# jinhan/tacotron2-vae

Hardware: AMD Instinct MI355X
Metric: mel-frames/s (train step, batch=6, 80-mel) (higher is better)
Workload: dtype f32; 1 GPU; configs[1]: Tacotron2-VAE fp32 train step (fwd+loss+bwd+clip+Adam), B=6/GPU fixed shape T_in=84 T_out=400, dropout on, random-init seed 1234; step_mode=hip-graph replay, decoder_forward=persistent, decoder_backward=persistent, startup_steps=43, global_batch=6, parallelism=dp1

## Files before the change

### tacotron2-vae_amd/csrc/conv_gemm.hip

```cpp
#include <stdlib.h>
#include <type_traits>
#include "t2v_common.h"
#include "t2v_kernels.h"
#include "t2v_ring.h"
#include "t2v_coop.h"
#include "t2v_x3.h"


#define CG_BM 64
#define CG_BN 64
#define CG_BK 32

struct ConvGemmArgs {
    const float* W;
    const float* X;
    const float* dY;
    const float* bias;
    float* Y;
    float* stat_part;
    int B, Cin, T, M, KS;
};

template <int MODE, int KS>
__global__ __launch_bounds__(256) void k_conv_gemm(ConvGemmArgs a) {
// ... 158 lines not shown
        if (second_ == 0u) return;
        if (tid == 0) __hip_atomic_store(a.ks_ctr + tile, 0u, __ATOMIC_RELAXED, __HIP_MEMORY_SCOPE_AGENT);
        const float* other = a.ks_part + (((1 - blockIdx.z) * ntile + tile) * 256 + tid) * (4 * NTW);
        float o[NTW][4];
#pragma unroll
        for (int n = 0; n < NTW; ++n)
#pragma unroll
            for (int r = 0; r < 4; ++r) o[n][r] = ld_sc1(other + 4 * n + r);
#pragma unroll
        for (int n = 0; n < NTW; ++n)
#pragma unroll
            for (int r = 0; r < 4; ++r) acc[n][r] += o[n][r];
    }
    float psum[4] = {0.f, 0.f, 0.f, 0.f}, psq[4] = {0.f, 0.f, 0.f, 0.f};
#pragma unroll
    for (int r = 0; r < 4; ++r) {
        const int m = m0 + 16 * wave + 4 * kq + r;
        if (m < a.M) {
            const float bv = a.bias ? a.bias[m] : 0.f;
            float* yrow = a.Y + ((size_t)bb * a.M + m) * a.T;
#pragma unroll
            for (int n = 0; n < NTW; ++n) {
                const int t = t0 + 16 * n + j;
                if (t < a.T) {
                    const float v = acc[n][r] + bv;
                    yrow[t] = v;
                    psum[r] += v;
                    psq[r] = fmaf(v, v, psq[r]);
                }
            }
        }
    }
    if (a.stat_part) {
#pragma unroll
        for (int r = 0; r < 4; ++r) {
            const float s1 = row16_sum(psum[r]), s2 = row16_sum(psq[r]);
            const int m = m0 + 16 * wave + 4 * kq + r;
            if (j == 0 && m < a.M) {
                float* dst = a.stat_part + ((size_t)blockIdx.x * a.M + m) * 2;
                dst[0] = s1;
                dst[1] = s2;
            }
        }
    }
}

template <int NTW>
__global__ __launch_bounds__(256) void k_conv5_fwd(ConvTiledArgs a) {
    constexpr int BN = 16 * NTW;
    constexpr int XW = BN + 4;
    constexpr int XS = BN == 32 ? 48 : BN <= 64 ? 80 : 112;
    constexpr int NX = (16 * XW + 255) / 256;
    __shared__ float As[2][CT_KT][CT_AS];
    __shared__ float Xs[2][16][XS];
    const int tid = threadIdx.x, wave = tid >> 6, lane = tid & 63;
    const int kq = lane >> 4, j = lane & 15;
    const int bb = blockIdx.x / a.tiles_per_item, t0 = (blockIdx.x % a.tiles_per_item) * BN;
    const int m0 = blockIdx.y * CT_BM;
    const int CK = a.Cin * 5;
    const int nkt_all = a.Cin / 16;
    const int kt0 = gridDim.z > 1 ? (int)blockIdx.z * (nkt_all / 2) : 0;
    const int nkt = gridDim.z > 1 ? (blockIdx.z == 0 ? nkt_all / 2 : nkt_all - nkt_all / 2) : nkt_all;

    const bool stamp = a.prof && tid == 0 && blockIdx.x == 0 && blockIdx.y == 0 && blockIdx.z == 0;
    if (stamp) { a.prof[0] = __builtin_readcyclecounter(); a.prof[2] = wall_clock64(); }
    float4 ra[5];
    float rx[NX];
    const int a_m = tid & 63, w4 = tid >> 6;
    const float* a_row = a.W + (size_t)min(m0 + a_m, a.M - 1) * CK + 4 * w4;
    int a_lds[20];
#pragma unroll
    for (int q = 0; q < 20; ++q) {
        const int k = 4 * w4 + 16 * (q >> 2) + (q & 3);
        const int c = k / 5, kx = k - 5 * c;
        a_lds[q] = (16 * kx + c) * CT_AS + a_m;
    }
    const float* x_item = a.X + (size_t)bb * a.Cin * a.T;
    int x_goff[NX], x_lds[NX];
    bool x_ok[NX];
#pragma unroll
    for (int i = 0; i < NX; ++i) {
        const int e = tid + 256 * i;
        const int c = min(e / XW, 15), jj = e - (e / XW) * XW;
        const int t = t0 - 2 + jj;
        x_ok[i] = e < 16 * XW && t >= 0 && t < a.T;
        x_goff[i] = c * a.T + min(max(t, 0), a.T - 1);
        x_lds[i] = e < 16 * XW ? c * XS + jj : -1;
    }
    auto load_one = [&](int kt, int q) {
        if (q < 5) {
            ra[q] = *(const float4*)(a_row + 80 * (kt0 + kt) + 16 * q);
        } else {
            const float v = x_item[(size_t)16 * (kt0 + kt) * a.T + x_goff[q - 5]];
            rx[q - 5] = x_ok[q - 5] ? v : 0.f;
        }
    };
    auto store_one = [&](int buf, int q) {
        if (q < 20) {
            const float4 v4 = ra[q >> 2];
            const float v = (q & 3) == 0 ? v4.x : (q & 3) == 1 ? v4.y : (q & 3) == 2 ? v4.z : v4.w;
            (&As[buf][0][0])[a_lds[q]] = v;
        } else if (q < 20 + NX) {
            if (x_lds[q - 20] >= 0) (&Xs[buf][0][0])[x_lds[q - 20]] = rx[q - 20];
        }
    };
    constexpr int NLOAD = 5 + NX, NSTORE = 20 + NX;
    constexpr int S_ST0 = 11;
    static_assert(NLOAD <= S_ST0 + 1 && NSTORE <= 3 * (20 - S_ST0), "side work must fit the k-steps");

    f32x4 acc[NTW];
#pragma unroll
    for (int n = 0; n < NTW; ++n) acc[n] = f32x4{0.f, 0.f, 0.f, 0.f};
#pragma unroll
    for (int q = 0; q < NLOAD; ++q) load_one(0, q);
#pragma unroll
    for (int q = 0; q < NSTORE; ++q) store_one(0, q);
    __syncthreads();
    for (int kt = 0; kt < nkt; ++kt) {
        const int buf = kt & 1;
        const int kn = min(kt + 1, nkt - 1);
        const float* ap = &As[buf][kq][16 * wave + j];
        const float* xp = &Xs[buf][kq][j];
        float av[2], bv[2][NTW];
        av[0] = ap[0];
#pragma unroll
        for (int n = 0; n < NTW; ++n) bv[0][n] = xp[16 * n];
#pragma unroll
        for (int s = 0; s < 20; ++s) {
            if (s < NLOAD) load_one(kn, s);
            if (s + 1 < 20) {
                av[(s + 1) & 1] = ap[4 * (s + 1) * CT_AS];
#pragma unroll
                for (int n = 0; n < NTW; ++n)
                    bv[(s + 1) & 1][n] = xp[4 * ((s + 1) & 3) * XS + 16 * n + ((s + 1) >> 2)];
            }
            __builtin_amdgcn_sched_barrier(0);
#pragma unroll
            for (int n = 0; n < NTW; ++n) acc[n] = mfma16x4(av[s & 1], bv[s & 1][n], acc[n]);
            __builtin_amdgcn_sched_barrier(0);
            if (s >= S_ST0) {
#pragma unroll
                for (int q = 3 * (s - S_ST0); q < 3 * (s - S_ST0) + 3; ++q) store_one(buf ^ 1, q);
                __builtin_amdgcn_sched_barrier(0);
            }
        }
        __syncthreads();
    }
    if (stamp) { a.prof[1] = __builtin_readcyclecounter(); a.prof[3] = wall_clock64(); }
    conv5_fwd_finish<NTW>(a, acc, bb, t0, m0);
}

#define CD_RING 3
#define CD_AS 84
__device__ float g_conv5_zero[4];

template <int NTW>
__global__ __launch_bounds__(256) void k_conv5_fwd_dma(ConvTiledArgs a) {
    constexpr int BN = 16 * NTW;
    constexpr int XW = BN + 4;
    constexpr int XS = BN == 32 ? 48 : BN <= 64 ? 80 : 112;
    constexpr int NXD = 16 * XS / 256;
    constexpr int G = 6 + NXD;
    constexpr int AST = CT_BM * CD_AS, STG = AST + 16 * XS;
    static_assert(16 * XS % 256 == 0 && AST % 256 == 0, "whole 64-lane requests");
    __shared__ __attribute__((aligned(16))) float lds_[CD_RING * STG];
    const unsigned lds0 = (unsigned)(unsigned long)(__attribute__((address_space(3))) void*)&lds_[0];
    const int tid = threadIdx.x, wave = __builtin_amdgcn_readfirstlane(tid >> 6), lane = tid & 63;
    const int kq = lane >> 4, j = lane & 15;
    const int bb = blockIdx.x / a.tiles_per_item, t0 = (blockIdx.x % a.tiles_per_item) * BN;
    const int m0 = blockIdx.y * CT_BM;
    const int CK = a.Cin * 5;
    const int nkt_all = a.Cin / 16;
    const int kt0 = gridDim.z > 1 ? (int)blockIdx.z * (nkt_all / 2) : 0;
    const int nkt = gridDim.z > 1 ? (blockIdx.z == 0 ? nkt_all / 2 : nkt_all - nkt_all / 2) : nkt_all;

    const bool stamp = a.prof && tid == 0 && blockIdx.x == 0 && blockIdx.y == 0 && blockIdx.z == 0;
    if (stamp) { a.prof[0] = __builtin_readcyclecounter(); a.prof[2] = wall_clock64(); }
    const float* a_ptr[6];
#pragma unroll
    for (int i = 0; i < 6; ++i) {
        const int u = 64 * min(wave + 4 * i, 20) + lane;
        const int row = u / 21, pc = u - 21 * row;
        a_ptr[i] = a.W + (size_t)min(m0 + row, a.M - 1) * CK + 80 * kt0 + 4 * min(pc, 19);
    }
    const float* x_ptr[NXD];
    size_t x_step[NXD];
#pragma unroll
    for (int i = 0; i < NXD; ++i) {
        const int e = 64 * (wave + 4 * i) + lane;
        const int c = e / XS, jj = e - c * XS;
        const int t = t0 - 2 + jj;
        const bool ok = jj < XW && t >= 0 && t < a.T;
        x_ptr[i] = ok ? a.X + ((size_t)bb * a.Cin + 16 * kt0 + c) * a.T + t : g_conv5_zero;
        x_step[i] = ok ? (size_t)16 * a.T : 0;
    }
    auto request = [&](unsigned dst, int q) {
        if (q < 5) {
            t2v_dma16(a_ptr[q], dst + 1024u * (unsigned)wave + 4096u * q);
            a_ptr[q] += 80;
        } else if (q == 5) {
            t2v_dma16(a_ptr[5], dst + 20480u);
            a_ptr[5] += 80;
        } else if (q < G) {
            t2v_dma4(x_ptr[q - 6], dst + 4u * AST + 256u * (unsigned)wave + 1024u * (q - 6));
            x_ptr[q - 6] += x_step[q - 6];
        }
    };

    f32x4 acc[NTW];
#pragma unroll
    for (int n = 0; n < NTW; ++n) acc[n] = f32x4{0.f, 0.f, 0.f, 0.f};
#pragma unroll
    for (int q = 0; q < G; ++q) request(lds0, q);
    if (nkt > 1) {
#pragma unroll
        for (int q = 0; q < G; ++q) request(lds0 + 4u * STG, q);
    }
    if (nkt > 1) t2v_wait_vmcnt<G>(); else t2v_wait_vmcnt<0>();
    __syncthreads();
    constexpr int CD_SYNC = 10;
    constexpr int TWO = G > 20 - CD_SYNC ? G - (20 - CD_SYNC) : 0;
    static_assert(G <= 2 * (20 - CD_SYNC) && (TWO == 0 || NTW >= 3), "a tile's requests fit the steps behind the barrier");
    const int lane_a = CD_AS * (16 * wave + j) + 5 * kq, lane_x = AST + kq * XS + j;
    float av[2], bv[2][NTW];
    auto fetch = [&](const float* ap, const float* xp, int s) {
        av[s & 1] = ap[20 * (s & 3) + (s >> 2)];
#pragma unroll
        for (int n = 0; n < NTW; ++n) bv[s & 1][n] = xp[4 * (s & 3) * XS + 16 * n + (s >> 2)];
    };
    auto tile = [&](auto more_c, const float* ap, const float* xp, const float* ap1, const float* xp1, unsigned dst2) {
        constexpr bool MORE = decltype(more_c)::value;
#pragma unroll
        for (int s = 0; s < 20; ++s) {
            if (s == CD_SYNC) {
                t2v_wait_vmcnt<0>();
                __syncthreads();
                __builtin_amdgcn_sched_barrier(0);
            }
            const int sr = s - CD_SYNC;
            const int q0 = !MORE || sr < 0 ? -1 : sr < TWO ? 2 * sr : sr + TWO;
            const int q1 = MORE && sr >= 0 && sr < TWO ? 2 * sr + 1 : -1;
#pragma unroll
            for (int n = 0; n < NTW; ++n) {
                acc[n] = mfma16x4(av[s & 1], bv[s & 1][n], acc[n]);
                __builtin_amdgcn_sched_barrier(0);
                if (n == 0) { if (s + 1 < 20) fetch(ap, xp, s + 1); else fetch(ap1, xp1, 0); }
                if (n == 1 && q0 >= 0 && q0 < G) request(dst2, q0);
                if (n == 2 && q1 >= 0) request(dst2, q1);
                __builtin_amdgcn_sched_barrier(0);
            }
        }
    };
    fetch(&lds_[lane_a], &lds_[lane_x], 0);
    int stg = 0;
    for (int kt = 0; kt < nkt; ++kt) {
        const int stg1 = stg == CD_RING - 1 ? 0 : stg + 1, stg2 = stg == 0 ? CD_RING - 1 : stg - 1;
        const float* ap = &lds_[stg * STG + lane_a];
        const float* xp = &lds_[stg * STG + lane_x];
        const float* ap1 = &lds_[stg1 * STG + lane_a];
        const float* xp1 = &lds_[stg1 * STG + lane_x];
        if (kt + 2 < nkt) tile(std::true_type{}, ap, xp, ap1, xp1, lds0 + 4u * (unsigned)(stg2 * STG));
        else tile(std::false_type{}, ap, xp, ap1, xp1, 0u);
        stg = stg1;
    }
    if (stamp) { a.prof[1] = __builtin_readcyclecounter(); a.prof[3] = wall_clock64(); }
    conv5_fwd_finish<NTW>(a, acc, bb, t0, m0);
}

template <int BT>
__global__ __launch_bounds__(256) void k_conv5_dw(ConvTiledArgs a) {
    constexpr int XW = BT + 4;
    constexpr int XS = (BT == 80) ? 100 : 116;
    constexpr int NA = BT / 16;
    constexpr int NX = (16 * XW + 255) / 256;
    __shared__ float As[2][BT][CT_AS];
    __shared__ float Xs[2][16][XS];
    const int tid = threadIdx.x, wave = tid >> 6, lane = tid & 63;
    const int kq = lane >> 4, j = lane & 15;
    const int c0 = blockIdx.x * 16, m0 = blockIdx.y * CT_BM;
    const int CK = a.Cin * 5;
    const int tiles = (a.T + BT - 1) / BT, nkt_all = a.B * tiles;
    const int per = (nkt_all + gridDim.z - 1) / gridDim.z;
    const int kt_lo = blockIdx.z * per, kt_hi = min(nkt_all, kt_lo + per);
    const bool vec = (a.T & 3) == 0;

    float4 ra[NA];
    float rx[NX];
    const int a_m = tid & 63;
    const bool a_ok = m0 + a_m < a.M;
    auto load_tiles = [&](int kt) {
        const int bb = kt / tiles, t0 = (kt - bb * tiles) * BT;
        const float* arow = a.dY + ((size_t)bb * a.M + (a_ok ? m0 + a_m : 0)) * a.T;
#pragma unroll
        for (int i = 0; i < NA; ++i) {
            const int t = t0 + 4 * ((tid >> 6) + 4 * i);
            float4 v = make_float4(0.f, 0.f, 0.f, 0.f);
            if (a_ok) {
                if (vec) {
                    if (t < a.T) v = *(const float4*)(arow + t);
                } else {
                    if (t < a.T) v.x = arow[t];
                    if (t + 1 < a.T) v.y = arow[t + 1];
                    if (t + 2 < a.T) v.z = arow[t + 2];
                    if (t + 3 < a.T) v.w = arow[t + 3];
                }
            }
            ra[i] = v;
        }
        const float* x_item = a.X + ((size_t)bb * a.Cin + c0) * a.T;
#pragma unroll
        for (int i = 0; i < NX; ++i) {
            const int e = tid + 256 * i;
            const int c = e / XW, jj = e - c * XW;
            const int t = t0 - 2 + jj;
            rx[i] = (c < 16 && t >= 0 && t < a.T) ? x_item[(size_t)c * a.T + t] : 0.f;
        }
    };
    auto store_tiles = [&](int buf) {
#pragma unroll
        for (int i = 0; i < NA; ++i) {
            const int k = 4 * ((tid >> 6) + 4 * i);
            As[buf][k][a_m] = ra[i].x;
            As[buf][k + 1][a_m] = ra[i].y;
            As[buf][k + 2][a_m] = ra[i].z;
            As[buf][k + 3][a_m] = ra[i].w;
        }
#pragma unroll
        for (int i = 0; i < NX; ++i) {
            const int e = tid + 256 * i;
            const int c = e / XW, jj = e - c * XW;
            if (c < 16) Xs[buf][c][jj] = rx[i];
        }
    };

    int boff[5];
#pragma unroll
    for (int n = 0; n < 5; ++n) {
        const int nl = 16 * n + j, c = nl / 5, kx = nl - 5 * c;
        boff[n] = c * XS + kx + kq;
    }
    f32x4 acc[5];
#pragma unroll
    for (int n = 0; n < 5; ++n) acc[n] = f32x4{0.f, 0.f, 0.f, 0.f};
    if (kt_lo < kt_hi) {
        load_tiles(kt_lo);
        store_tiles(0);
    }
    __syncthreads();
    for (int kt = kt_lo; kt < kt_hi; ++kt) {
        const int buf = (kt - kt_lo) & 1;
        if (kt + 1 < kt_hi) load_tiles(kt + 1);
        const float* ap = &As[buf][kq][16 * wave + j];
        const float* xp = &Xs[buf][0][0];
        float av[2], bv[2][5];
        av[0] = ap[0];
#pragma unroll
        for (int n = 0; n < 5; ++n) bv[0][n] = xp[boff[n]];
#pragma unroll
        for (int s = 0; s < BT / 4; ++s) {
            if (s + 1 < BT / 4) {
                av[(s + 1) & 1] = ap[4 * (s + 1) * CT_AS];
#pragma unroll
                for (int n = 0; n < 5; ++n) bv[(s + 1) & 1][n] = xp[boff[n] + 4 * (s + 1)];
            }
            __builtin_amdgcn_sched_barrier(0);
#pragma unroll
            for (int n = 0; n < 5; ++n) acc[n] = mfma16x4(av[s & 1], bv[s & 1][n], acc[n]);
            __builtin_amdgcn_sched_barrier(0);
        }
        if (kt + 1 < kt_hi) store_tiles(buf ^ 1);
        __syncthreads();
    }
#pragma unroll
    for (int r = 0; r < 4; ++r) {
        const int m = m0 + 16 * wave + 4 * kq + r;
        if (m < a.M) {
            float* drow = a.Y + (size_t)blockIdx.z * a.M * CK + (size_t)m * CK + 5 * c0;
#pragma unroll
            for (int n = 0; n < 5; ++n) drow[16 * n + j] = acc[n][r];
        }
    }
}

#define CB_RS 24

__global__ void k_conv5_pack_bf16(const float* __restrict__ W, unsigned short* __restrict__ Wp, int M, int Cin, int flipT) {
    const int R = flipT ? Cin : M, Cc = flipT ? M : Cin;
    const size_t i = (size_t)blockIdx.x * blockDim.x + threadIdx.x;
    if (i >= (size_t)R * Cc * 5) return;
    const int c16 = i & 15, kx = (i >> 4) % 5;
    const size_t rc = (i >> 4) / 5;
    const int cb = rc % (Cc / 16), r = rc / (Cc / 16);
    const int cc = 16 * cb + c16;
    const float v = flipT ? W[((size_t)cc * Cin + r) * 5 + (4 - kx)] : W[((size_t)r * Cin + cc) * 5 + kx];
    const __bf16 b = (__bf16)v;
    Wp[i] = *(const unsigned short*)&b;
}

struct ConvBf16Args {
    const unsigned short* Wp;
    const float* X;
    const float* bias;
    float* Y;
    float* stat_part;
    int B, Cin, T, M, tiles_per_item;
};

template <int NTW>
__global__ __launch_bounds__(256) void k_conv5_fwd_bf16(ConvBf16Args a) {
    constexpr int BN = 16 * NTW;
    constexpr int XW = BN + 4;
    constexpr int NXP = (8 * XW + 255) / 256;
    __shared__ __attribute__((aligned(16))) unsigned short As[2][5][CT_BM][CB_RS];
    __shared__ __attribute__((aligned(16))) unsigned short Xt[2][XW][CB_RS];
    const int tid = threadIdx.x, wave = tid >> 6, lane = tid & 63;
    const int kq = lane >> 4, j = lane & 15;
    const int bb = blockIdx.x / a.tiles_per_item, t0 = (blockIdx.x % a.tiles_per_item) * BN;
    const int m0 = blockIdx.y * CT_BM;
    const int ncb = a.Cin / 16;

    uint4 ra[3];
    const unsigned short* a_src[3];
    int a_lds[3];
#pragma unroll
    for (int i = 0; i < 3; ++i) {
        const int q = tid + 256 * i;
        const int row = min(q / 10, CT_BM - 1), ch = q - (q / 10) * 10;
        a_src[i] = a.Wp + (size_t)min(m0 + row, a.M - 1) * ncb * 80 + ch * 8;
        a_lds[i] = q < 640 ? (((ch >> 1) * CT_BM + row) * CB_RS + 8 * (ch & 1)) : -1;
    }
    float rx[NXP][2];
    const float* x_item = a.X + (size_t)bb * a.Cin * a.T;
    int x_goff[NXP], x_lds[NXP];
    bool x_ok[NXP];
#pragma unroll
    for (int i = 0; i < NXP; ++i) {
        const int e = tid + 256 * i;
        const int cp = min(e / XW, 7), pos = e - (e / XW) * XW;
        const int t = t0 - 2 + pos;
        x_ok[i] = e < 8 * XW && t >= 0 && t < a.T;
        x_goff[i] = 2 * cp * a.T + min(max(t, 0), a.T - 1);
        x_lds[i] = e < 8 * XW ? pos * CB_RS + 2 * cp : -1;
    }
    auto load_tiles = [&](int kt) {
#pragma unroll
        for (int i = 0; i < 3; ++i) ra[i] = *(const uint4*)(a_src[i] + 80 * kt);
#pragma unroll
        for (int i = 0; i < NXP; ++i) {
            const float* px = x_item + (size_t)16 * kt * a.T + x_goff[i];
            const float v0 = px[0], v1 = px[a.T];
            rx[i][0] = x_ok[i] ? v0 : 0.f;
            rx[i][1] = x_ok[i] ? v1 : 0.f;
        }
    };
    auto store_tiles = [&](int buf) {
#pragma unroll
        for (int i = 0; i < 3; ++i)
            if (a_lds[i] >= 0) *(uint4*)(&As[buf][0][0][0] + a_lds[i]) = ra[i];
#pragma unroll
        for (int i = 0; i < NXP; ++i)
            if (x_lds[i] >= 0) *(unsigned*)(&Xt[buf][0][0] + x_lds[i]) = t2v_pack_bf16x2(rx[i][0], rx[i][1]);
    };

    f32x4 acc[NTW];
#pragma unroll
    for (int n = 0; n < NTW; ++n) acc[n] = f32x4{0.f, 0.f, 0.f, 0.f};
    load_tiles(0);
    store_tiles(0);
    __syncthreads();
    for (int kt = 0; kt < ncb; ++kt) {
        const int buf = kt & 1;
        load_tiles(min(kt + 1, ncb - 1));
#pragma unroll
        for (int kx = 0; kx < 5; ++kx) {
            const t2v_s16x4 av = *(const t2v_s16x4*)&As[buf][kx][16 * wave + j][4 * kq];
#pragma unroll
            for (int n = 0; n < NTW; ++n) {
                const t2v_s16x4 bv = *(const t2v_s16x4*)&Xt[buf][16 * n + j + kx][4 * kq];
                acc[n] = __builtin_amdgcn_mfma_f32_16x16x16bf16_1k(av, bv, acc[n], 0, 0, 0);
            }
        }
        store_tiles(buf ^ 1);
        __syncthreads();
    }

    float psum[4] = {0.f, 0.f, 0.f, 0.f}, psq[4] = {0.f, 0.f, 0.f, 0.f};
#pragma unroll
    for (int r = 0; r < 4; ++r) {
        const int m = m0 + 16 * wave + 4 * kq + r;
        if (m < a.M) {
            const float bv = a.bias ? a.bias[m] : 0.f;
            float* yrow = a.Y + ((size_t)bb * a.M + m) * a.T;
#pragma unroll
            for (int n = 0; n < NTW; ++n) {
                const int t = t0 + 16 * n + j;
                if (t < a.T) {
                    const float v = acc[n][r] + bv;
                    yrow[t] = v;
                    psum[r] += v;
                    psq[r] = fmaf(v, v, psq[r]);
                }
            }
        }
    }
    if (a.stat_part) {
#pragma unroll
        for (int r = 0; r < 4; ++r) {
            const float s1 = row16_sum(psum[r]), s2 = row16_sum(psq[r]);
            const int m = m0 + 16 * wave + 4 * kq + r;
            if (j == 0 && m < a.M) {
                float* dst = a.stat_part + ((size_t)blockIdx.x * a.M + m) * 2;
                dst[0] = s1;
                dst[1] = s2;
            }
        }
    }
}

#define CB2_RS 40
template <int NTW>
__global__ __launch_bounds__(256) void k_conv5_fwd_bf16k32(ConvBf16Args a) {
    constexpr int BN = 16 * NTW;
    constexpr int XW = BN + 4;
    constexpr int NXP = (16 * XW + 255) / 256;
    __shared__ __attribute__((aligned(16))) unsigned short As[2][5][CT_BM][CB2_RS];
    __shared__ __attribute__((aligned(16))) unsigned short Xt[2][XW][CB2_RS];
    const int tid = threadIdx.x, wave = tid >> 6, lane = tid & 63;
    const int kq = lane >> 4, j = lane & 15;
    const int bb = blockIdx.x / a.tiles_per_item, t0 = (blockIdx.x % a.tiles_per_item) * BN;
    const int m0 = blockIdx.y * CT_BM;
    const int ncb = a.Cin / 16, nkt = a.Cin / 32;

// ... 300 lines not shown
    int ksplit;
    int dw_splits;
    int stat_blocks;
    int dw_scratch_floats;
};
static ConvRoute conv_route(int op, int B, int Cin, int T, int Cout, int KS, bool bf16, bool w_aligned) {
    ConvRoute r;
    r.op = op; r.B = B; r.T = T; r.KS = KS;
    r.Cin = op == CONV_OP_DX ? Cout : Cin;
    r.M = op == CONV_OP_DX ? Cin : Cout;
    r.family = r.fallback = CONV_K_GEMM;
    r.tile = 0; r.ksplit = 1; r.dw_splits = 1; r.dw_scratch_floats = 0;
    r.stat_blocks = op == CONV_OP_DW ? 0 : (B * T + CG_BN - 1) / CG_BN;
    if (KS != 5 || r.Cin % 16) return r;
    if (op == CONV_OP_DW) {
        r.family = bf16 ? CONV_K_DW_BF16 : CONV_K_DW;
        r.tile = conv5_dw_bt(T);
        r.dw_splits = conv5_dw_splits(B, Cin, T, Cout, r.tile, bf16);
        r.dw_scratch_floats = r.dw_splits > 1 ? r.dw_splits * Cout * Cin * 5 : 0;
        return r;
    }
    int ks = 1;
    const int BN = conv5_pick_bn_ks(T, B, r.M, r.Cin, &ks);
    r.tile = BN / 16;
    r.stat_blocks = B * ((T + BN - 1) / BN);
    if (bf16) {
        static const int k32 = getenv("T2V_CONV_BF16_K32") ? atoi(getenv("T2V_CONV_BF16_K32")) : 1;
        r.family = k32 && r.Cin % 32 == 0 ? CONV_K_BF16K32 : CONV_K_BF16;
    } else {
        static const int staging = getenv("T2V_CONV_STAGING") ? atoi(getenv("T2V_CONV_STAGING")) : 1;
        r.family = staging && w_aligned ? CONV_K_FWD_DMA : CONV_K_FWD;
        r.ksplit = ks;
    }
    if (t2v_conv5_planes_ok(B, r.Cin, T, r.M, KS, bf16 ? 1 : 3)) {
        r.fallback = r.family;
        r.family = bf16 ? CONV_K_PLANE1 : CONV_K_X3;
        r.ksplit = 1;
        r.stat_blocks = t2v_conv5_x3_stat_blocks(B, T);
    }
    return r;
}

__global__ void k_conv_flip_weight(const float* __restrict__ W, float* __restrict__ Wt, int M, int Cin, int KS) {
    const int i = blockIdx.x * blockDim.x + threadIdx.x;
    if (i >= M * Cin * KS) return;
    const int k = i % KS, c = (i / KS) % Cin, m = i / (KS * Cin);
    Wt[((size_t)c * M + m) * KS + (KS - 1 - k)] = W[i];
}

struct ConvFlipBatch { const float* W[16]; float* Wt[16]; int M[16]; int Cin[16]; int n; int KS; };
__global__ void k_conv_flip_weight_batched(ConvFlipBatch f) {
    const int l = blockIdx.y;
    const int M = f.M[l], Cin = f.Cin[l], KS = f.KS;
    const float* __restrict__ W = f.W[l];
    float* __restrict__ Wt = f.Wt[l];
    const int n = M * Cin * KS;
    for (int i = blockIdx.x * blockDim.x + threadIdx.x; i < n; i += gridDim.x * blockDim.x) {
        const int k = i % KS, c = (i / KS) % Cin, m = i / (KS * Cin);
        Wt[((size_t)c * M + m) * KS + (KS - 1 - k)] = W[i];
    }
}

extern "C" int t2v_conv1d_flip_weights(const float* const* W, float* const* Wt, const int* Cout, const int* Cin, int KS,
                                       int n, void* stream_) {
    hipStream_t stream = (hipStream_t)stream_;
    if (!W || !Wt || !Cout || !Cin || n < 1 || n > 16 || KS < 1) return T2V_ERR_ARG;
    ConvFlipBatch f;
    f.n = n; f.KS = KS;
    int mx = 0;
    for (int i = 0; i < n; ++i) {
        if (!W[i] || !Wt[i] || Cout[i] < 1 || Cin[i] < 1) return T2V_ERR_ARG;
        f.W[i] = W[i]; f.Wt[i] = Wt[i]; f.M[i] = Cout[i]; f.Cin[i] = Cin[i];
        mx = max(mx, Cout[i] * Cin[i] * KS);
    }
    const int bx = min(1024, (mx + 1023) / 1024);
    k_conv_flip_weight_batched<<<dim3(bx, n), 256, 0, stream>>>(f);
    return t2v_check_launch();
}

static std::atomic<long long> g_conv5_staged_launches{0};
extern "C" long long t2v_conv1d_staged_launches(void) { return g_conv5_staged_launches.load(std::memory_order_relaxed); }

#define T2V_CONV_GEMM(MODE, W_, X_, DY_, BIAS_, Y_, STAT_)                                              \
    ConvGemmArgs g;                                                                                     \
    g.W = W_; g.X = X_; g.dY = DY_; g.bias = BIAS_; g.Y = Y_; g.stat_part = STAT_;                      \
    g.B = r.B; g.Cin = r.Cin; g.T = r.T; g.M = r.M; g.KS = r.KS;                                        \
    const dim3 gg(((MODE == 0 ? r.B * r.T : r.Cin * r.KS) + CG_BN - 1) / CG_BN, (r.M + CG_BM - 1) / CG_BM);   \
    if (r.KS == 5) k_conv_gemm<MODE, 5><<<gg, 256, 0, stream>>>(g);                                     \
    else if (r.KS == 3) k_conv_gemm<MODE, 3><<<gg, 256, 0, stream>>>(g);                                \
    else return T2V_ERR_DIMS;                                                                           \
    return T2V_OK
#define T2V_CONV5_NTW(KERNEL)                                       \
    switch (r.tile) {                                               \
    case 2: KERNEL<2><<<grid, 256, 0, stream>>>(a); break;          \
    case 3: KERNEL<3><<<grid, 256, 0, stream>>>(a); break;          \
    case 4: KERNEL<4><<<grid, 256, 0, stream>>>(a); break;          \
    case 5: KERNEL<5><<<grid, 256, 0, stream>>>(a); break;          \
    default: KERNEL<6><<<grid, 256, 0, stream>>>(a);                \
    }
static int conv_launch(const ConvRoute& r, const float* W, const float* X, const float* bias, float* Y, float* stat_part,
                       unsigned short* Wp, hipStream_t stream) {
    const int B = r.B, Cin = r.Cin, T = r.T, M = r.M, BN = 16 * r.tile;
    const bool dx = r.op == CONV_OP_DX;
    int family = r.family;
    if (family == CONV_K_X3) return t2v_conv5_x3_run(W, X, bias, Y, stat_part, B, Cin, T, M, stream, 3);
    if (family == CONV_K_PLANE1 && !dx) return t2v_conv5_x3_run(W, X, bias, Y, stat_part, B, Cin, T, M, stream, 1);
    if (family == CONV_K_PLANE1) {
        float* wt = conv_ks_scratch((size_t)M * Cin * 5);
        if (wt) {
            k_conv_flip_weight<<<(M * Cin * 5 + 255) / 256, 256, 0, stream>>>(W, wt, Cin, M, 5);
            return t2v_conv5_x3_run(wt, X, bias, Y, stat_part, B, Cin, T, M, stream, 1);
        }
        family = r.fallback;
    }
    if (family == CONV_K_FWD || family == CONV_K_FWD_DMA) {
        ConvTiledArgs a;
        a.W = W; a.X = X; a.dY = nullptr; a.bias = bias; a.Y = Y; a.stat_part = stat_part;
        a.B = B; a.Cin = Cin; a.T = T; a.M = M; a.tiles_per_item = (T + BN - 1) / BN;
        a.prof = g_t2v_prof;
        a.ks_part = nullptr; a.ks_ctr = nullptr;
        dim3 grid(B * a.tiles_per_item, (M + CT_BM - 1) / CT_BM);
        if (r.ksplit == 2) {
            const long ntile = (long)grid.x * grid.y;
            a.ks_part = conv_ks_scratch((size_t)2 * ntile * 256 * 4 * r.tile);
            a.ks_ctr = a.ks_part ? t2v_arrival_counters((int)ntile) : nullptr;
            if (a.ks_part && a.ks_ctr) grid.z = 2; else a.ks_part = nullptr;
        }
        if (family == CONV_K_FWD_DMA) {
            g_conv5_staged_launches.fetch_add(1, std::memory_order_relaxed);
            T2V_CONV5_NTW(k_conv5_fwd_dma)
        } else {
            T2V_CONV5_NTW(k_conv5_fwd)
        }
        return T2V_OK;
    }
    if (family == CONV_K_BF16 || family == CONV_K_BF16K32) {
        const size_t n = (size_t)M * Cin * 5;
        k_conv5_pack_bf16<<<(unsigned)((n + 255) / 256), 256, 0, stream>>>(W, Wp, dx ? Cin : M, dx ? M : Cin, dx ? 1 : 0);
        ConvBf16Args a;
        a.Wp = Wp; a.X = X; a.bias = bias; a.Y = Y; a.stat_part = stat_part;
        a.B = B; a.Cin = Cin; a.T = T; a.M = M; a.tiles_per_item = (T + BN - 1) / BN;
        dim3 grid(B * a.tiles_per_item, (M + CT_BM - 1) / CT_BM);
        if (family == CONV_K_BF16K32) { T2V_CONV5_NTW(k_conv5_fwd_bf16k32) } else { T2V_CONV5_NTW(k_conv5_fwd_bf16) }
        return T2V_OK;
    }
    T2V_CONV_GEMM(0, W, X, nullptr, bias, Y, stat_part);
}
#undef T2V_CONV5_NTW

static int conv_dw_launch(const ConvRoute& r, const float* X, const float* dY, float* dW, float* dw_scratch, hipStream_t stream) {
    if (r.family != CONV_K_GEMM) {
        const int ns = r.dw_splits;
        if (ns > 1 && !dw_scratch) return T2V_ERR_ARG;
        ConvTiledArgs a;
        a.W = nullptr; a.X = X; a.dY = dY; a.bias = nullptr; a.Y = ns > 1 ? dw_scratch : dW; a.stat_part = nullptr;
        a.B = r.B; a.Cin = r.Cin; a.T = r.T; a.M = r.M; a.tiles_per_item = 0;
        a.prof = nullptr; a.ks_part = nullptr; a.ks_ctr = nullptr;
        dim3 grid(r.Cin / 16, (r.M + CT_BM - 1) / CT_BM, ns);
        if (r.family == CONV_K_DW_BF16) {
            if (r.tile == 80) k_conv5_dw_bf16<80><<<grid, 256, 0, stream>>>(a);
            else k_conv5_dw_bf16<96><<<grid, 256, 0, stream>>>(a);
        } else if (r.tile == 80) k_conv5_dw<80><<<grid, 256, 0, stream>>>(a);
        else k_conv5_dw<96><<<grid, 256, 0, stream>>>(a);
        if (ns > 1) {
            const int n = r.M * r.Cin * 5;
            k_conv5_dw_reduce<<<(n + 255) / 256, 256, 0, stream>>>(dw_scratch, dW, n, ns);
        }
        return T2V_OK;
    }
    T2V_CONV_GEMM(1, nullptr, X, dY, nullptr, dW, nullptr);
}
#undef T2V_CONV_GEMM

extern "C" int t2v_conv1d_fwd(const float* W, const float* X, const float* bias, float* Y, float* stat_part,
                              int B, int Cin, int T, int Cout, int KS, void* stream_) {
    if (!W || !X || !Y || B < 1 || Cin < 1 || T < 1 || Cout < 1 || KS < 1 || !(KS & 1)) return T2V_ERR_ARG;
    const ConvRoute r = conv_route(CONV_OP_FWD, B, Cin, T, Cout, KS, false, ((size_t)W & 15) == 0);
    const int rc = conv_launch(r, W, X, bias, Y, stat_part, nullptr, (hipStream_t)stream_);
    return rc != T2V_OK ? rc : t2v_check_launch();
}

extern "C" int t2v_conv1d_stat_blocks(int B, int T, int Cin, int Cout, int KS) {
    return conv_route(CONV_OP_FWD, B, Cin, T, Cout, KS, false, true).stat_blocks;
}
extern "C" int t2v_conv1d_stat_blocks_bf16(int B, int T, int Cin, int Cout, int KS) {
    return conv_route(CONV_OP_FWD, B, Cin, T, Cout, KS, true, true).stat_blocks;
}
extern "C" int t2v_conv1d_dw_scratch_floats(int B, int Cin, int T, int Cout, int KS) {
    return conv_route(CONV_OP_DW, B, Cin, T, Cout, KS, true, true).dw_scratch_floats;
}
extern "C" int t2v_conv1d_takes_x3(int B, int Cin, int T, int Cout, int KS, int bf16) {
    const int family = conv_route(CONV_OP_FWD, B, Cin, T, Cout, KS, bf16 != 0, true).family;
    return family == CONV_K_X3 || family == CONV_K_PLANE1 ? 1 : 0;
}
static_assert(CONV_OP_FWD == T2V_CONV_OP_FWD && CONV_OP_DX == T2V_CONV_OP_DX && CONV_OP_DW == T2V_CONV_OP_DW, "t2vae.h");
static_assert(CONV_K_GEMM == T2V_CONV_ROUTE_GEMM && CONV_K_FWD == T2V_CONV_ROUTE_FWD && CONV_K_FWD_DMA == T2V_CONV_ROUTE_FWD_DMA &&
              CONV_K_X3 == T2V_CONV_ROUTE_X3 && CONV_K_BF16 == T2V_CONV_ROUTE_BF16 && CONV_K_BF16K32 == T2V_CONV_ROUTE_BF16K32 &&
              CONV_K_PLANE1 == T2V_CONV_ROUTE_PLANE1 && CONV_K_DW == T2V_CONV_ROUTE_DW && CONV_K_DW_BF16 == T2V_CONV_ROUTE_DW_BF16 &&
              CONV_K_DW_BF16 + 1 == T2V_CONV_ROUTES, "t2vae.h");
extern "C" int t2v_conv1d_route(int op, int B, int Cin, int T, int Cout, int KS, int bf16, int w_mod16, int* fallback, int* tile,
                                int* ksplit, int* dw_splits, int* stat_blocks, int* dw_scratch_floats, int* plane_splits,
                                int* plane_chunk) {
    if (op < CONV_OP_FWD || op > CONV_OP_DW || B < 1 || Cin < 1 || T < 1 || Cout < 1 || KS < 1 || !(KS & 1)) return T2V_ERR_ARG;
    const ConvRoute r = conv_route(op, B, Cin, T, Cout, KS, bf16 != 0, (w_mod16 & 15) == 0);
    if (bf16 && r.family == CONV_K_GEMM) return T2V_ERR_DIMS;
    if (fallback) *fallback = r.fallback;
    if (tile) *tile = r.tile;
    if (ksplit) *ksplit = r.ksplit;
    if (dw_splits) *dw_splits = r.dw_splits;
    if (stat_blocks) *stat_blocks = r.stat_blocks;
    if (dw_scratch_floats) *dw_scratch_floats = r.dw_scratch_floats;
    int chunk = 0;
    const bool planes = r.family == CONV_K_X3 || r.family == CONV_K_PLANE1;
    const int nz = planes ? t2v_conv5_x3_splits(B, r.Cin, T, r.M, r.family == CONV_K_X3 ? 3 : 1, &chunk) : 0;
    if (plane_splits) *plane_splits = nz;
    if (plane_chunk) *plane_chunk = chunk;
    return r.family;
}
extern "C" const char* t2v_conv1d_route_name(int route) {
    static const char* const names[T2V_CONV_ROUTES] = {"gemm", "fwd", "fwd_dma", "x3", "bf16", "bf16k32", "plane1", "dw", "dw_bf16"};
    return route >= 0 && route < T2V_CONV_ROUTES ? names[route] : "?";
}

extern "C" int t2v_conv1d_bwd(const float* W, const float* X, const float* dY, float* dX, float* dW, float* Wt_scratch,
                              float* dw_scratch, int B, int Cin, int T, int Cout, int KS, void* stream_) {
    hipStream_t stream = (hipStream_t)stream_;
    if (!X || !dY || B < 1 || Cin < 1 || T < 1 || Cout < 1 || KS < 1 || !(KS & 1)) return T2V_ERR_ARG;
    if (dX) {
        if (!Wt_scratch) return T2V_ERR_ARG;
        const int n = Cout * Cin * KS;
        if (W) k_conv_flip_weight<<<(n + 255) / 256, 256, 0, stream>>>(W, Wt_scratch, Cout, Cin, KS);
        const ConvRoute r = conv_route(CONV_OP_DX, B, Cin, T, Cout, KS, false, ((size_t)Wt_scratch & 15) == 0);
        const int rc = conv_launch(r, Wt_scratch, dY, nullptr, dX, nullptr, nullptr, stream);
        if (rc != T2V_OK) return rc;
    }
    if (dW) {
        const int rc = conv_dw_launch(conv_route(CONV_OP_DW, B, Cin, T, Cout, KS, false, true), X, dY, dW, dw_scratch, stream);
        if (rc != T2V_OK) return rc;
    }
    return t2v_check_launch();
}

extern "C" int t2v_conv1d_fwd_bf16(const float* W, const float* X, const float* bias, float* Y, float* stat_part,
                                   void* Wp_scratch, int B, int Cin, int T, int Cout, int KS, void* stream_) {
    if (!W || !X || !Y || !Wp_scratch || B < 1 || Cin < 1 || T < 1 || Cout < 1) return T2V_ERR_ARG;
    const ConvRoute r = conv_route(CONV_OP_FWD, B, Cin, T, Cout, KS, true, true);
    if (r.family == CONV_K_GEMM) return T2V_ERR_DIMS;
    const int rc = conv_launch(r, W, X, bias, Y, stat_part, (unsigned short*)Wp_scratch, (hipStream_t)stream_);
    return rc != T2V_OK ? rc : t2v_check_launch();
}

extern "C" int t2v_conv1d_bwd_bf16(const float* W, const float* X, const float* dY, float* dX, float* dW,
                                   void* Wp_scratch, float* dw_scratch, int B, int Cin, int T, int Cout, int KS,
                                   void* stream_) {
    hipStream_t stream = (hipStream_t)stream_;
    if (!X || !dY || B < 1 || Cin < 1 || T < 1 || Cout < 1) return T2V_ERR_ARG;
    const ConvRoute rw = conv_route(CONV_OP_DW, B, Cin, T, Cout, KS, true, true);
    if (rw.family == CONV_K_GEMM) return T2V_ERR_DIMS;
    if (dX) {
        const ConvRoute rx = conv_route(CONV_OP_DX, B, Cin, T, Cout, KS, true, true);
        if (rx.family == CONV_K_GEMM) return T2V_ERR_DIMS;
        if (!W || !Wp_scratch) return T2V_ERR_ARG;
        const int rc = conv_launch(rx, W, dY, nullptr, dX, nullptr, (unsigned short*)Wp_scratch, stream);
        if (rc != T2V_OK) return rc;
    }
    if (dW) {
        const int rc = conv_dw_launch(rw, X, dY, dW, dw_scratch, stream);
        if (rc != T2V_OK) return rc;
    }
    return t2v_check_launch();
}
```

Baseline: 231,200 mel-frames/s.

## Add wide-LDS conv5 weight-gradient kernel with interleaved staging stores

Adds a new k_conv5_dw_wide kernel and makes it the default for the fp32 conv weight-gradient path. The kernel reads float4 operands from LDS, reusing each X fragment across all five taps by sliding a window over eight values, instead of issuing scalar LDS loads per tap. The next tile's stores to LDS are spread between MFMAs in the last two groups, and bounds checks go through a zero-pointer redirect. It also adds ablation macros, profiling timestamps and an env switch, which add a little overhead and complexity, plus an alignment check on the old path.

Result: no change. 231,700 mel-frames/s (median of 5 runs) (+0.2%).

```diff
diff --git a/tacotron2-vae_amd/csrc/conv_gemm.hip b/tacotron2-vae_amd/csrc/conv_gemm.hip
--- a/tacotron2-vae_amd/csrc/conv_gemm.hip
+++ b/tacotron2-vae_amd/csrc/conv_gemm.hip
@@ -334,7 +334,7 @@
 
 #define CD_RING 3
 #define CD_AS 84
-__device__ float g_conv5_zero[4];
+__device__ __attribute__((aligned(16))) float g_conv5_zero[4];
 
 template <int NTW>
 __global__ __launch_bounds__(256) void k_conv5_fwd_dma(ConvTiledArgs a) {
@@ -449,6 +449,9 @@
     conv5_fwd_finish<NTW>(a, acc, bb, t0, m0);
 }
 
+#ifndef T2V_DW_ABLATE
+#define T2V_DW_ABLATE 0
+#endif
 template <int BT>
 __global__ __launch_bounds__(256) void k_conv5_dw(ConvTiledArgs a) {
     constexpr int XW = BT + 4;
@@ -464,7 +467,8 @@
     const int tiles = (a.T + BT - 1) / BT, nkt_all = a.B * tiles;
     const int per = (nkt_all + gridDim.z - 1) / gridDim.z;
     const int kt_lo = blockIdx.z * per, kt_hi = min(nkt_all, kt_lo + per);
-    const bool vec = (a.T & 3) == 0;
+    const bool vec = (a.T & 3) == 0 && ((size_t)a.dY & 15) == 0;
+    const bool stamp = a.prof && tid == 0 && blockIdx.x == 0 && blockIdx.y == 0 && blockIdx.z == 0;
 
     float4 ra[NA];
     float rx[NX];
@@ -529,9 +533,10 @@
         store_tiles(0);
     }
     __syncthreads();
+    if (stamp) { a.prof[0] = __builtin_readcyclecounter(); a.prof[2] = wall_clock64(); }
     for (int kt = kt_lo; kt < kt_hi; ++kt) {
         const int buf = (kt - kt_lo) & 1;
-        if (kt + 1 < kt_hi) load_tiles(kt + 1);
+        if (T2V_DW_ABLATE != 3 && kt + 1 < kt_hi) load_tiles(kt + 1);
         const float* ap = &As[buf][kq][16 * wave + j];
         const float* xp = &Xs[buf][0][0];
         float av[2], bv[2][5];
@@ -541,18 +546,31 @@
 #pragma unroll
         for (int s = 0; s < BT / 4; ++s) {
             if (s + 1 < BT / 4) {
-                av[(s + 1) & 1] = ap[4 * (s + 1) * CT_AS];
-#pragma unroll
-                for (int n = 0; n < 5; ++n) bv[(s + 1) & 1][n] = xp[boff[n] + 4 * (s + 1)];
+                if (T2V_DW_ABLATE == 1) {
+                    av[(s + 1) & 1] = av[s & 1];
+#pragma unroll
+                    for (int n = 0; n < 5; ++n) bv[(s + 1) & 1][n] = bv[s & 1][n];
+                } else {
+                    av[(s + 1) & 1] = ap[4 * (s + 1) * CT_AS];
+#pragma unroll
+                    for (int n = 0; n < 5; ++n) bv[(s + 1) & 1][n] = xp[boff[n] + 4 * (s + 1)];
+                }
             }
             __builtin_amdgcn_sched_barrier(0);
 #pragma unroll
             for (int n = 0; n < 5; ++n) acc[n] = mfma16x4(av[s & 1], bv[s & 1][n], acc[n]);
             __builtin_amdgcn_sched_barrier(0);
         }
-        if (kt + 1 < kt_hi) store_tiles(buf ^ 1);
+        if (T2V_DW_ABLATE != 2 && kt + 1 < kt_hi) store_tiles(buf ^ 1);
+        if (T2V_DW_ABLATE == 2) {
+#pragma unroll
+            for (int i = 0; i < NA; ++i) asm volatile("" ::"v"(ra[i].x), "v"(ra[i].y), "v"(ra[i].z), "v"(ra[i].w));
+#pragma unroll
+            for (int i = 0; i < NX; ++i) asm volatile("" ::"v"(rx[i]));
+        }
         __syncthreads();
     }
+    if (stamp) { a.prof[1] = __builtin_readcyclecounter(); a.prof[3] = wall_clock64(); }
 #pragma unroll
     for (int r = 0; r < 4; ++r) {
         const int m = m0 + 16 * wave + 4 * kq + r;
@@ -560,6 +578,140 @@
             float* drow = a.Y + (size_t)blockIdx.z * a.M * CK + (size_t)m * CK + 5 * c0;
 #pragma unroll
             for (int n = 0; n < 5; ++n) drow[16 * n + j] = acc[n][r];
+        }
+    }
+}
+
+template <int BT, bool VEC>
+__global__ __launch_bounds__(256) void k_conv5_dw_wide(ConvTiledArgs a) {
+    constexpr int NG = BT / 16;
+    constexpr int NQ = BT / 4;
+    constexpr int NA = NQ * CT_BM / 256;
+    constexpr int XW = BT + 4;
+    constexpr int RS = BT + 8;
+    constexpr int NX = (16 * XW + 255) / 256;
+    constexpr int AST = CT_BM * RS, STG = AST + 16 * RS;
+    static_assert(NQ * CT_BM % 256 == 0 && RS % 16 == 8 && RS >= XW, "staging plan / bank rule");
+    __shared__ __attribute__((aligned(16))) float lds_[2 * STG];
+    const int tid = threadIdx.x, wave = tid >> 6, lane = tid & 63;
+    const int kq = lane >> 4, j = lane & 15;
+    const int c0 = blockIdx.x * 16, m0 = blockIdx.y * CT_BM;
+    const int CK = a.Cin * 5;
+    const int tiles = (a.T + BT - 1) / BT, nkt_all = a.B * tiles;
+    const int per = (nkt_all + gridDim.z - 1) / gridDim.z;
+    const int kt_lo = blockIdx.z * per, kt_hi = min(nkt_all, kt_lo + per);
+    const bool stamp = a.prof && tid == 0 && blockIdx.x == 0 && blockIdx.y == 0 && blockIdx.z == 0;
+
+    int a_row[NA], a_t[NA], a_lds[NA];
+#pragma unroll
+    for (int i = 0; i < NA; ++i) {
+        const int e = tid + 256 * i, row = e / NQ, q = e - row * NQ;
+        const bool ok = m0 + row < a.M;
+        a_row[i] = (ok ? row : 0) * a.T;
+        a_t[i] = ok ? 4 * q : 1 << 30;
+        a_lds[i] = row * RS + 4 * q;
+    }
+    int x_row[NX], x_j[NX], x_lds[NX];
+#pragma unroll
+    for (int i = 0; i < NX; ++i) {
+        const int e = tid + 256 * i, c = e / XW, jj = e - c * XW;
+        x_row[i] = min(c, 15) * a.T;
+        x_j[i] = c < 16 ? jj - 2 : -(1 << 30);
+        x_lds[i] = c < 16 ? AST + c * RS + jj : AST + XW;
+    }
+    const float* const zero = g_conv5_zero;
+    float4 ra[NA];
+    float rx[NX];
+    auto load_tiles = [&](int kt) {
+        const int bb = kt / tiles, t0 = (kt - bb * tiles) * BT;
+        const float* ab = a.dY + ((size_t)bb * a.M + m0) * a.T;
+#pragma unroll
+        for (int i = 0; i < NA; ++i) {
+            const int t = t0 + a_t[i];
+            const float* p = ab + a_row[i];
+            if (VEC) {
+                const float4 v = *(const float4*)(t < a.T ? p + t : zero);
+                ra[i] = v;
+            } else {
+                const float v0 = *(t < a.T ? p + t : zero), v1 = *(t + 1 < a.T ? p + t + 1 : zero);
+                const float v2 = *(t + 2 < a.T ? p + t + 2 : zero), v3 = *(t + 3 < a.T ? p + t + 3 : zero);
+                ra[i] = make_float4(v0, v1, v2, v3);
+            }
+        }
+        const float* xb = a.X + ((size_t)bb * a.Cin + c0) * a.T;
+#pragma unroll
+        for (int i = 0; i < NX; ++i) {
+            const int t = t0 + x_j[i];
+            rx[i] = *((unsigned)t < (unsigned)a.T ? xb + x_row[i] + t : zero);
+        }
+    };
+    auto store_one = [&](int buf, int q) {
+        if (q < NA) *(float4*)&lds_[buf * STG + a_lds[q]] = ra[q];
+        else if (q < NA + NX) lds_[buf * STG + x_lds[q - NA]] = rx[q - NA];
+    };
+    constexpr int NSTORE = NA + NX;
+    static_assert(NSTORE <= 20 && NG >= 2, "the stores are dealt out two MFMAs apart over the last two groups");
+
+    f32x4 acc[5];
+#pragma unroll
+    for (int n = 0; n < 5; ++n) acc[n] = f32x4{0.f, 0.f, 0.f, 0.f};
+    if (kt_lo < kt_hi) {
+        load_tiles(kt_lo);
+#pragma unroll
+        for (int q = 0; q < NSTORE; ++q) store_one(0, q);
+    }
+    __syncthreads();
+    if (stamp) { a.prof[0] = __builtin_readcyclecounter(); a.prof[2] = wall_clock64(); }
+    const int lane_a = (16 * wave + j) * RS + 4 * kq, lane_x = AST + j * RS + 4 * kq;
+    float4 av[2], bl[2], bh[2];
+    auto fetch = [&](const float* base, int g) {
+        av[g & 1] = *(const float4*)(base + lane_a + 16 * g);
+        bl[g & 1] = *(const float4*)(base + lane_x + 16 * g);
+        bh[g & 1] = *(const float4*)(base + lane_x + 16 * g + 4);
+    };
+    if (T2V_DW_ABLATE == 1) { fetch(lds_, 0); av[1] = av[0]; bl[1] = bl[0]; bh[1] = bh[0]; }
+    for (int kt = kt_lo; kt < kt_hi; ++kt) {
+        const int buf = (kt - kt_lo) & 1;
+        const float* base = lds_ + buf * STG;
+        if (T2V_DW_ABLATE != 3) load_tiles(min(kt + 1, kt_hi - 1));
+        if (T2V_DW_ABLATE != 1) fetch(base, 0);
+#pragma unroll
+        for (int g = 0; g < NG; ++g) {
+            if (T2V_DW_ABLATE != 1 && g + 1 < NG) fetch(base, g + 1);
+            __builtin_amdgcn_sched_barrier(0);
+            const float4 a4 = av[g & 1], l4 = bl[g & 1], h4 = bh[g & 1];
+            const float ar[4] = {a4.x, a4.y, a4.z, a4.w};
+            const float xr[8] = {l4.x, l4.y, l4.z, l4.w, h4.x, h4.y, h4.z, h4.w};
+#pragma unroll
+            for (int i = 0; i < 4; ++i)
+#pragma unroll
+                for (int kx = 0; kx < 5; ++kx) {
+                    acc[kx] = mfma16x4(ar[i], xr[i + kx], acc[kx]);
+                    if (g >= NG - 2) {
+                        const int p = 20 * (g - (NG - 2)) + 5 * i + kx;
+                        __builtin_amdgcn_sched_barrier(0);
+                        if (T2V_DW_ABLATE != 2 && (p & 1) && (p >> 1) < NSTORE) store_one(buf ^ 1, p >> 1);
+                        __builtin_amdgcn_sched_barrier(0);
+                    }
+                }
+            __builtin_amdgcn_sched_barrier(0);
+        }
+        if (T2V_DW_ABLATE == 2) {
+#pragma unroll
+            for (int i = 0; i < NA; ++i) asm volatile("" ::"v"(ra[i].x), "v"(ra[i].y), "v"(ra[i].z), "v"(ra[i].w));
+#pragma unroll
+            for (int i = 0; i < NX; ++i) asm volatile("" ::"v"(rx[i]));
+        }
+        __syncthreads();
+    }
+    if (stamp) { a.prof[1] = __builtin_readcyclecounter(); a.prof[3] = wall_clock64(); }
+#pragma unroll
+    for (int r = 0; r < 4; ++r) {
+        const int m = m0 + 16 * wave + 4 * kq + r;
+        if (m < a.M) {
+            float* d = a.Y + (size_t)blockIdx.z * a.M * CK + (size_t)m * CK + 5 * (c0 + j);
+#pragma unroll
+            for (int kx = 0; kx < 5; ++kx) d[kx] = acc[kx][r];
         }
     }
 }
@@ -1166,16 +1318,24 @@
     if (r.family != CONV_K_GEMM) {
         const int ns = r.dw_splits;
         if (ns > 1 && !dw_scratch) return T2V_ERR_ARG;
+        if (r.T >= 1 << 30) return T2V_ERR_DIMS;
         ConvTiledArgs a;
         a.W = nullptr; a.X = X; a.dY = dY; a.bias = nullptr; a.Y = ns > 1 ? dw_scratch : dW; a.stat_part = nullptr;
         a.B = r.B; a.Cin = r.Cin; a.T = r.T; a.M = r.M; a.tiles_per_item = 0;
-        a.prof = nullptr; a.ks_part = nullptr; a.ks_ctr = nullptr;
+        a.prof = r.family == CONV_K_DW ? g_t2v_prof : nullptr; a.ks_part = nullptr; a.ks_ctr = nullptr;
         dim3 grid(r.Cin / 16, (r.M + CT_BM - 1) / CT_BM, ns);
+        static const int wide = getenv("T2V_CONV_DW") ? atoi(getenv("T2V_CONV_DW")) : 1;
         if (r.family == CONV_K_DW_BF16) {
             if (r.tile == 80) k_conv5_dw_bf16<80><<<grid, 256, 0, stream>>>(a);
             else k_conv5_dw_bf16<96><<<grid, 256, 0, stream>>>(a);
-        } else if (r.tile == 80) k_conv5_dw<80><<<grid, 256, 0, stream>>>(a);
-        else k_conv5_dw<96><<<grid, 256, 0, stream>>>(a);
+        } else if (!wide) {
+            if (r.tile == 80) k_conv5_dw<80><<<grid, 256, 0, stream>>>(a);
+            else k_conv5_dw<96><<<grid, 256, 0, stream>>>(a);
+        } else if (r.T % 4 == 0 && ((size_t)dY & 15) == 0) {
+            if (r.tile == 80) k_conv5_dw_wide<80, true><<<grid, 256, 0, stream>>>(a);
+            else k_conv5_dw_wide<96, true><<<grid, 256, 0, stream>>>(a);
+        } else if (r.tile == 80) k_conv5_dw_wide<80, false><<<grid, 256, 0, stream>>>(a);
+        else k_conv5_dw_wide<96, false><<<grid, 256, 0, stream>>>(a);
         if (ns > 1) {
             const int n = r.M * r.Cin * 5;
             k_conv5_dw_reduce<<<(n + 255) / 256, 256, 0, stream>>>(dw_scratch, dW, n, ns);
```
